# mayursharma/PageRank-using-Apache-Spark

Measured on AMD Instinct MI355X. Metric: PageRank GTEPS/iter + % HBM roofline, R-MAT scale-26 at 1/2/4/8 MI355X, higher is better.
Workload: dtype f64

## Files before the change

### pagerank-using-apache-spark_amd/csrc/pr_spmv.h

```cpp
#pragma once

#include <climits>

#include "pr_device.h"
#include "pr_internal.h"

namespace pr {

__device__ __forceinline__ double dc_from_slots(const double *cin, const SlotPos &sp) {
  double dc = 0.0;
  for (int p = 0; p < sp.n; ++p) dc = __dadd_rn(dc, cin[sp.pos[p]]);
  return dc;
}

__device__ __forceinline__ double affine(double S, double tdc, double teleport, double damping) {
  return __dadd_rn(teleport, __dmul_rn(damping, __dadd_rn(S, tdc)));
}

typedef int pr_v4i __attribute__((ext_vector_type(4)));
typedef int pr_v2i __attribute__((ext_vector_type(2)));
typedef pr_v4i pr_v4i_alias __attribute__((may_alias));
typedef uint32_t pr_u32_alias __attribute__((may_alias));
typedef double pr_f64_alias __attribute__((may_alias));

template <int PT, bool NT>
__device__ __forceinline__ void load_cols(const int32_t *__restrict__ p, int32_t (&ci)[PT]) {
  static_assert(PT % 4 == 0, "PT must be a multiple of 4");
  const pr_v4i *q = reinterpret_cast<const pr_v4i *>(p);
#pragma unroll
  for (int k = 0; k < PT / 4; ++k) {
    pr_v4i x;
    if constexpr (NT) x = __builtin_nontemporal_load(q + k);
    else x = q[k];
    ci[4 * k + 0] = x.x;
    ci[4 * k + 1] = x.y;
    ci[4 * k + 2] = x.z;
    ci[4 * k + 3] = x.w;
  }
}

template <int PT, bool NT, bool TELE>
__global__ __launch_bounds__(kThreads) void k_spmv_units(
    const Unit *__restrict__ units, const int64_t *__restrict__ rowptr,
    const int32_t *__restrict__ colp, const double *__restrict__ cin, double *__restrict__ cout,
    double *__restrict__ r, const uint32_t *__restrict__ rowinfo, double *__restrict__ piece_part,
    double2 *__restrict__ unit_part, SlotPos sp, int64_t S_pad, double n_vertices, double teleport,
    double damping, const double *__restrict__ tele) {
  __shared__ double rowsum[kUnitRows];
  __shared__ int32_t lrp[kUnitRows + 1];
  __shared__ double red[kThreads / kWave];
  __shared__ double2 red2[kThreads / kWave];
  __shared__ int32_t wrow_first[kThreads / kWave], wrow_last[kThreads / kWave];
  __shared__ double wval_last[kThreads / kWave];

  const int t = threadIdx.x, lane = lane_id(), w = wave_id();
  const Unit u = units[blockIdx.x];
  const int n = unit_n(u);
  const int i0 = t * PT;
  const bool stream = u.meta >= 0;
  const int nr = stream ? u.meta : 0;
  const int32_t r0 = u.r0;

  int32_t ci[PT];
  if (i0 < n) {
    load_cols<PT, NT>(colp + (int64_t)u.p8 * 8 + i0, ci);
  } else {
#pragma unroll
    for (int j = 0; j < PT; ++j) ci[j] = 0;
  }
  int64_t rp_t = 0;
  double rold0 = 0.0, tele0 = teleport;
  uint32_t info0 = 0;
  if (stream) {
    if (t <= nr) rp_t = rowptr[r0 + t];
    if (t < nr) {
      rold0 = r[(int64_t)r0 + t];
      info0 = rowinfo[(int64_t)r0 + t];
      if constexpr (TELE) tele0 = tele[(int64_t)r0 + t];
    }
  }

  double v[PT];
#pragma unroll
  for (int j = 0; j < PT; ++j) v[j] = (i0 + j < n) ? cin[ci[j]] : 0.0;

  if (!stream) {
    double acc = 0.0;
#pragma unroll
    for (int j = 0; j < PT; ++j) acc = __dadd_rn(acc, v[j]);
    acc = block_sum<kThreads>(acc, red);
    if (t == 0) {
      piece_part[-u.meta - 1] = acc;
      unit_part[blockIdx.x] = make_double2(0.0, 0.0);
    }
    return;
  }

  const int64_t e0 = rowptr[r0];
  if (t <= nr) lrp[t] = (int32_t)(rp_t - e0);
  for (int k = t + kThreads; k <= nr; k += kThreads) lrp[k] = (int32_t)(rowptr[r0 + k] - e0);
  const double tdc = dc_from_slots(cin, sp) / n_vertices;
  __syncthreads();

  int carry_row = -1, first_row = -1;
  double carry_val = 0.0, first_sum = 0.0;
  if (i0 < n) {
    int lo = 0, hi = nr + 1;
    while (lo < hi) {
      const int mid = (lo + hi) >> 1;
      if (lrp[mid] <= i0) lo = mid + 1;
      else hi = mid;
    }
    int cur = lo - 1;
    const int kstart = cur;
    const bool started_before = lrp[cur] < i0;
    int next_end = lrp[cur + 1];
    double acc = 0.0;
    bool open = false;
#pragma unroll
    for (int j = 0; j < PT; ++j) {
      if (i0 + j < n) {
        acc = __dadd_rn(acc, v[j]);
        open = true;
        if (i0 + j + 1 == next_end) {
          if (cur == kstart && started_before) {
            first_row = cur;
            first_sum = acc;
          } else {
            rowsum[cur] = acc;
          }
          acc = 0.0;
          open = false;
          ++cur;
          while (cur < nr && lrp[cur + 1] == lrp[cur]) ++cur;
          next_end = (cur < nr) ? lrp[cur + 1] : INT_MAX;
        }
      }
    }
    if (open) {
      carry_row = cur;
      carry_val = acc;
    }
  }

  int srow = carry_row;
  double sval = carry_val;
#pragma unroll
  for (int off = 1; off < kWave; off <<= 1) {
    const int prow = __shfl_up(srow, off, kWave);
    const double pval = __shfl_up(sval, off, kWave);
    if (lane >= off && srow >= 0 && prow == srow) sval = __dadd_rn(pval, sval);
  }
  const int lane0_row = __shfl(carry_row, 0, kWave);
  if (lane == kWave - 1) {
    wrow_last[w] = srow;
    wval_last[w] = sval;
    wrow_first[w] = lane0_row;
  }
  __syncthreads();
  int prow_in = -1;
  double pval_in = 0.0;
  for (int ww = 0; ww < w; ++ww) {
    const int rl = wrow_last[ww];
    const bool full = (rl >= 0) && (wrow_first[ww] == rl);
    if (full && prow_in == rl) {
      pval_in = __dadd_rn(pval_in, wval_last[ww]);
    } else {
      prow_in = rl;
      pval_in = (rl >= 0) ? wval_last[ww] : 0.0;
    }
  }
  if (srow >= 0 && srow == prow_in && lane0_row == srow) sval = __dadd_rn(pval_in, sval);
  int erow = __shfl_up(srow, 1, kWave);
  double eval = __shfl_up(sval, 1, kWave);
  if (lane == 0) {
    erow = prow_in;
    eval = pval_in;
  }
  if (first_row >= 0) rowsum[first_row] = (erow == first_row) ? __dadd_rn(eval, first_sum) : first_sum;
  __syncthreads();

  double dcp = 0.0, l1p = 0.0;
  for (int k = t; k < nr; k += kThreads) {
    const int64_t vtx = (int64_t)r0 + k;
    const double rold = (k == t) ? rold0 : r[vtx];
    const uint32_t info = (k == t) ? info0 : rowinfo[vtx];
    if (info & kRowHole) continue;
    const double S = (lrp[k + 1] > lrp[k]) ? rowsum[k] : rold;
    double tv = teleport;
    if constexpr (TELE) tv = (k == t) ? tele0 : tele[vtx];
    const double rn = affine(S, tdc, tv, damping);
    r[vtx] = rn;
    const uint32_t d = info & kRowDegMask;
    if (d > 0) cout[vtx] = __ddiv_rn(rn, (double)d);
    else if (info & kRowSink) dcp = __dadd_rn(dcp, rn);
    l1p = __dadd_rn(l1p, fabs(rn - rold));
  }
  const double2 part = block_sum2<kThreads>(make_double2(dcp, l1p), red2);
  if (t == 0) unit_part[blockIdx.x] = part;
}


template <int CTRL>
__device__ __forceinline__ double dpp_f64(double x) {
  const pr_v2i v = __builtin_bit_cast(pr_v2i, x);
  pr_v2i r;
  r.x = __builtin_amdgcn_update_dpp(0, v.x, CTRL, 0xF, 0xF, true);
  r.y = __builtin_amdgcn_update_dpp(0, v.y, CTRL, 0xF, 0xF, true);
  return __builtin_bit_cast(double, r);
}

template <int CTRL>
__device__ __forceinline__ int dpp_i32(int x) {
  return __builtin_amdgcn_update_dpp(0, x, CTRL, 0xF, 0xF, true);
}

__device__ __forceinline__ int wave_incl_scan_i32(int x) {
  const int row = lane_id() >> 4;
  x += dpp_i32<0x111>(x);
  x += dpp_i32<0x112>(x);
  x += dpp_i32<0x114>(x);
  x += dpp_i32<0x118>(x);
  int p = dpp_i32<0x142>(x);
  if (row == 1 || row == 3) x += p;
  p = dpp_i32<0x143>(x);
  if (row >= 2) x += p;
  return x;
}

__device__ __forceinline__ int wave_incl_max_i32(int x) {
  const int row = lane_id() >> 4;
  x = max(x, dpp_i32<0x111>(x));
  x = max(x, dpp_i32<0x112>(x));
  x = max(x, dpp_i32<0x114>(x));
  x = max(x, dpp_i32<0x118>(x));
  int p = dpp_i32<0x142>(x);
  if (row == 1 || row == 3) x = max(x, p);
  p = dpp_i32<0x143>(x);
  if (row >= 2) x = max(x, p);
  return x;
}

struct WaveCodes {
  uint32_t c[kWavePT];
};

__device__ __forceinline__ void wave_unit_codes(const Unit &u, const uint32_t *__restrict__ colh, WaveCodes &w) {
  const __amdgpu_buffer_rsrc_t rs =
      __builtin_amdgcn_make_buffer_rsrc((void *)(colh + (int64_t)u.p8 * 8), 0, u.n * 4, 0x00020000);
  const int base = lane_id() * kWavePT * 4;
#pragma unroll
  for (int q = 0; q < kWavePT / 4; ++q) {
    const pr_v4i x = __builtin_bit_cast(pr_v4i, __builtin_amdgcn_raw_buffer_load_b128(rs, base + 16 * q, 0, 2));
    w.c[4 * q + 0] = (uint32_t)x.x;
    w.c[4 * q + 1] = (uint32_t)x.y;
    w.c[4 * q + 2] = (uint32_t)x.z;
    w.c[4 * q + 3] = (uint32_t)x.w;
  }
}

struct WaveCodesC20 {
  uint32_t w[kWavePT / 2];
  uint32_t s;
};
__device__ __forceinline__ void wave_unit_codes(const Unit &u, const uint16_t *__restrict__ code16,
                                                const uint32_t *__restrict__ cside, WaveCodesC20 &w) {
  const __amdgpu_buffer_rsrc_t rm =
      __builtin_amdgcn_make_buffer_rsrc((void *)(code16 + (int64_t)u.p8 * 8), 0, u.n * 2, 0x00020000);
  const __amdgpu_buffer_rsrc_t rsd =
      __builtin_amdgcn_make_buffer_rsrc((void *)(cside + (int64_t)u.p8), 0, u.n / 2, 0x00020000);
  const pr_v4i x = __builtin_bit_cast(pr_v4i, __builtin_amdgcn_raw_buffer_load_b128(rm, lane_id() * 16, 0, 2));
  w.w[0] = (uint32_t)x.x;
  w.w[1] = (uint32_t)x.y;
  w.w[2] = (uint32_t)x.z;
  w.w[3] = (uint32_t)x.w;
  w.s = __builtin_amdgcn_raw_buffer_load_b32(rsd, lane_id() * 4, 0, 2);
}

struct WaveCodesC24 {
  uint32_t w[kWavePT / 2];
  uint64_t s;
};
__device__ __forceinline__ void wave_unit_codes(const Unit &u, const uint16_t *__restrict__ code16,
                                                const uint64_t *__restrict__ cside, WaveCodesC24 &w) {
  const __amdgpu_buffer_rsrc_t rm =
      __builtin_amdgcn_make_buffer_rsrc((void *)(code16 + (int64_t)u.p8 * 8), 0, u.n * 2, 0x00020000);
  const __amdgpu_buffer_rsrc_t rsd =
      __builtin_amdgcn_make_buffer_rsrc((void *)(cside + (int64_t)u.p8), 0, u.n, 0x00020000);
  const pr_v4i x = __builtin_bit_cast(pr_v4i, __builtin_amdgcn_raw_buffer_load_b128(rm, lane_id() * 16, 0, 2));
  w.w[0] = (uint32_t)x.x;
  w.w[1] = (uint32_t)x.y;
  w.w[2] = (uint32_t)x.z;
  w.w[3] = (uint32_t)x.w;
  w.s = __builtin_bit_cast(uint64_t, __builtin_amdgcn_raw_buffer_load_b64(rsd, lane_id() * 8, 0, 2));
}

__device__ __forceinline__ uint32_t end_marks(const WaveCodes &w) {
  uint32_t endm = 0;
#pragma unroll
  for (int j = 0; j < kWavePT; ++j) endm |= (w.c[j] & 1u) << j;
  return endm;
}
__device__ __forceinline__ uint32_t end_marks(const WaveCodesC20 &w) { return w.s & 0xFFu; }
__device__ __forceinline__ uint32_t end_marks(const WaveCodesC24 &w) { return (uint32_t)w.s & 0xFFu; }

struct LaneMeta {
  uint32_t endm;
  int excl;
  bool c[6];
};
__device__ __forceinline__ LaneMeta derive_meta(uint32_t endm) {
  LaneMeta m;
  m.endm = endm;
  const int t = lane_id(), r = t & 15, row = t >> 4;
  const int last1 = wave_incl_max_i32(endm ? t + 1 : 0);
  const int d = t + 1 - last1;
  const int dr = min(d, r);
#pragma unroll
  for (int s = 0; s < 4; ++s) m.c[s] = dr >= (1 << s);
  m.c[4] = (row & 1) && d > r;
  m.c[5] = row >= 2 && d > t - 32;
  const int cnt = __builtin_popcount(endm);
  m.excl = wave_incl_scan_i32(cnt) - cnt;
  return m;
}

struct ClassSrc {
  __amdgpu_buffer_rsrc_t crs;
  uint32_t zb, hb;
  const uint32_t *tbl;
};

template <bool PIECE>
__device__ __forceinline__ uint32_t cold_offset(uint32_t b8, const ClassSrc &cs) {
  if constexpr (PIECE) return piece_cold_offset(b8, cs.hb, cs.tbl);
  else return b8 - cs.hb;
}

#ifndef PR_GATHER_AUX
#define PR_GATHER_AUX 0
#endif
#ifndef PR_HOT_DIAG
#define PR_HOT_DIAG 0
#endif

template <bool PIECE>
__device__ __forceinline__ void wave_unit_gather(const WaveCodes &w, const double *hot, const ClassSrc &cs,
                                                 double (&v)[kWavePT]) {
#pragma unroll
  for (int j = 0; j < kWavePT; ++j) {
    const uint32_t c = w.c[j] & ~1u;
    const uint32_t la = (int32_t)c < 0 ? 0u : c;
    const double a = *reinterpret_cast<const double *>(reinterpret_cast<const char *>(hot) + la);
    const uint32_t go = c ^ kEntGlobal;
    const double b = __builtin_bit_cast(double, __builtin_amdgcn_raw_buffer_load_b64(cs.crs, go, 0, PR_GATHER_AUX));
    v[j] = __dadd_rn(a, b);
  }
}
template <bool PIECE>
__device__ __forceinline__ void wave_unit_gather(const WaveCodesC20 &w, const double *hot, const ClassSrc &cs,
                                                 double (&v)[kWavePT]) {
#pragma unroll
  for (int j = 0; j < kWavePT; ++j) {
    const uint32_t lo = (j & 1) ? (w.w[j >> 1] >> 16) : (w.w[j >> 1] & 0xFFFFu);
    const uint32_t idx = lo | (((w.s >> (8 + 3 * j)) & 7u) << 16);
    const uint32_t b8 = idx << 3;
    const uint32_t la = min(b8, cs.zb);
    const double a = *reinterpret_cast<const double *>(reinterpret_cast<const char *>(hot) + la);
#if PR_HOT_DIAG == 1
    const double b = __builtin_bit_cast(double, __builtin_amdgcn_raw_buffer_load_b64(cs.crs, cold_offset<PIECE>(b8, cs) | kEntGlobal, 0, PR_GATHER_AUX));
#elif PR_HOT_DIAG == 2 || PR_HOT_DIAG == 6
    const double b = 0.0;
#elif PR_HOT_DIAG == 3
    const uint32_t off = cold_offset<PIECE>(b8, cs);
    const double b = __dadd_rn(__builtin_bit_cast(double, __builtin_amdgcn_raw_buffer_load_b64(cs.crs, off, 0, PR_GATHER_AUX)),
                               __builtin_bit_cast(double, __builtin_amdgcn_raw_buffer_load_b64(cs.crs, off | kEntGlobal, 0, PR_GATHER_AUX)));
#else
    const double b = __builtin_bit_cast(double, __builtin_amdgcn_raw_buffer_load_b64(cs.crs, cold_offset<PIECE>(b8, cs), 0, PR_GATHER_AUX));
#endif
    v[j] = __dadd_rn(a, b);
  }
}

template <bool PIECE>
__device__ __forceinline__ void entry_addr(const WaveCodes &w, int j, const ClassSrc &, uint32_t &la, uint32_t &go) {
  const uint32_t c = w.c[j] & ~1u;
  la = (int32_t)c < 0 ? 0u : c;
  go = c ^ kEntGlobal;
}
template <bool PIECE>
__device__ __forceinline__ void entry_addr(const WaveCodesC20 &w, int j, const ClassSrc &cs, uint32_t &la, uint32_t &go) {
  const uint32_t lo = (j & 1) ? (w.w[j >> 1] >> 16) : (w.w[j >> 1] & 0xFFFFu);
  const uint32_t b8 = (lo | (((w.s >> (8 + 3 * j)) & 7u) << 16)) << 3;
  la = min(b8, cs.zb);
  go = cold_offset<PIECE>(b8, cs);
}
template <bool PIECE>
__device__ __forceinline__ void entry_addr(const WaveCodesC24 &w, int j, const ClassSrc &cs, uint32_t &la, uint32_t &go) {
  const uint32_t lo = (j & 1) ? (w.w[j >> 1] >> 16) : (w.w[j >> 1] & 0xFFFFu);
  const uint32_t b8 = (lo | ((uint32_t)(w.s >> (8 + 4 * j)) & 15u) << 16) << 3;
  la = min(b8, cs.zb);
  go = cold_offset<PIECE>(b8, cs);
}

static_assert(kStageSlots >= 2 * kWave, "the compact gather window holds 128 values (256 offsets)");
template <bool PIECE, class WC>
__device__ __forceinline__ void wave_unit_gather_compact(const WC &w, const double *hot, const ClassSrc &cs,
                                                         double (&v)[kWavePT], double *win) {
  uint32_t off[kWavePT], la[kWavePT];
  uint32_t coldm = 0u;
#pragma unroll
  for (int j = 0; j < kWavePT; ++j) {
    entry_addr<PIECE>(w, j, cs, la[j], off[j]);
    coldm |= ((int32_t)off[j] >= 0 ? 1u : 0u) << j;
  }
#pragma unroll
  for (int j = 0; j < kWavePT; ++j) v[j] = *reinterpret_cast<const double *>(reinterpret_cast<const char *>(hot) + la[j]);
  const int cnt = __builtin_popcount(coldm);
  const int incl = wave_incl_scan_i32(cnt);
  const int excl = incl - cnt, total = __builtin_amdgcn_readlane(incl, kWave - 1);
  const int lane = lane_id();
  pr_u32_alias *win32 = reinterpret_cast<pr_u32_alias *>(win);
  pr_f64_alias *winf = reinterpret_cast<pr_f64_alias *>(win);
  for (int base = 0; base < total; base += 4 * kWave) {
    int rk = excl - base;
#pragma unroll
    for (int j = 0; j < kWavePT; ++j) {
      const bool c = (coldm >> j) & 1u;
      if (c && (uint32_t)rk < (uint32_t)(4 * kWave)) win32[rk] = off[j];
      rk += c ? 1 : 0;
    }
    const int n = min(4 * kWave, total - base);
    const uint32_t a0 = lane < n ? win32[lane] : kEntGlobal;
    const uint32_t a1 = lane + kWave < n ? win32[lane + kWave] : kEntGlobal;
    const uint32_t a2 = lane + 2 * kWave < n ? win32[lane + 2 * kWave] : kEntGlobal;
    const uint32_t a3 = lane + 3 * kWave < n ? win32[lane + 3 * kWave] : kEntGlobal;
    const double g0 = __builtin_bit_cast(double, __builtin_amdgcn_raw_buffer_load_b64(cs.crs, a0, 0, PR_GATHER_AUX));
    double g1 = 0.0, g2 = 0.0, g3 = 0.0;
    if (n > kWave) g1 = __builtin_bit_cast(double, __builtin_amdgcn_raw_buffer_load_b64(cs.crs, a1, 0, PR_GATHER_AUX));
    if (n > 2 * kWave) g2 = __builtin_bit_cast(double, __builtin_amdgcn_raw_buffer_load_b64(cs.crs, a2, 0, PR_GATHER_AUX));
    if (n > 3 * kWave) g3 = __builtin_bit_cast(double, __builtin_amdgcn_raw_buffer_load_b64(cs.crs, a3, 0, PR_GATHER_AUX));
    winf[lane] = g0;
    if (n > kWave) winf[lane + kWave] = g1;
    rk = excl - base;
#pragma unroll
    for (int j = 0; j < kWavePT; ++j) {
      const bool c = (coldm >> j) & 1u;
      if (c && (uint32_t)rk < (uint32_t)(2 * kWave)) v[j] = winf[rk];
      rk += c ? 1 : 0;
    }
    if (n > 2 * kWave) {
      winf[lane] = g2;
      if (n > 3 * kWave) winf[lane + kWave] = g3;
      rk = excl - base - 2 * kWave;
#pragma unroll
      for (int j = 0; j < kWavePT; ++j) {
        const bool c = (coldm >> j) & 1u;
        if (c && (uint32_t)rk < (uint32_t)(2 * kWave)) v[j] = winf[rk];
        rk += c ? 1 : 0;
      }
    }
  }
}

template <bool PIECE>
__device__ __forceinline__ void wave_unit_gather(const WaveCodesC24 &w, const double *hot, const ClassSrc &cs,
                                                 double (&v)[kWavePT]) {
#pragma unroll
  for (int j = 0; j < kWavePT; ++j) {
    const uint32_t lo = (j & 1) ? (w.w[j >> 1] >> 16) : (w.w[j >> 1] & 0xFFFFu);
    const uint32_t idx = lo | ((uint32_t)(w.s >> (8 + 4 * j)) & 15u) << 16;
    const uint32_t b8 = idx << 3;
    const uint32_t la = min(b8, cs.zb);
    const double a = *reinterpret_cast<const double *>(reinterpret_cast<const char *>(hot) + la);
    const double b = __builtin_bit_cast(double, __builtin_amdgcn_raw_buffer_load_b64(cs.crs, cold_offset<PIECE>(b8, cs), 0, PR_GATHER_AUX));
    v[j] = __dadd_rn(a, b);
  }
}

__device__ __forceinline__ void wave_segmented_sums(const LaneMeta &m, const double (&v)[kWavePT],
                                                    double (&sv)[kWavePT], double *carry) {
  double acc = 0.0;
#pragma unroll
  for (int j = 0; j < kWavePT; ++j) {
    acc = __dadd_rn(acc, v[j]);
    sv[j] = acc;
    if (m.endm & (1u << j)) acc = 0.0;
  }
  double a = acc, p;
  p = dpp_f64<0x111>(a);
  if (m.c[0]) a = __dadd_rn(p, a);
  p = dpp_f64<0x112>(a);
  if (m.c[1]) a = __dadd_rn(p, a);
  p = dpp_f64<0x114>(a);
  if (m.c[2]) a = __dadd_rn(p, a);
  p = dpp_f64<0x118>(a);
  if (m.c[3]) a = __dadd_rn(p, a);
  p = dpp_f64<0x142>(a);
  if (m.c[4]) a = __dadd_rn(p, a);
  p = dpp_f64<0x143>(a);
  if (m.c[5]) a = __dadd_rn(p, a);
  *carry = dpp_f64<0x138>(a);
}

__device__ __forceinline__ void stage_segment_sums(const LaneMeta &m, const double (&sv)[kWavePT], double carry,
                                                   int base, double *stage) {
  int e = m.excl - base;
#pragma unroll
  for (int j = 0; j < kWavePT; ++j) {
    const bool end = (m.endm >> j) & 1u;
    if (end && e >= 0 && e < kStageSlots) stage[e] = sv[j];
    e += end ? 1 : 0;
  }
  const int e0 = m.excl - base;
  if (m.endm != 0u && e0 >= 0 && e0 < kStageSlots) stage[e0] = __dadd_rn(carry, stage[e0]);
}


struct UnitSums {
  LaneMeta m;
  double sv[kWavePT];
  double carry;
};

template <class WC>
__device__ __forceinline__ bool wave_unit_sums(const Unit &u, const WC &w, const double (&v)[kWavePT],
                                               double *__restrict__ piece_part, UnitSums &r) {
  if (u.meta < 0) {
    double acc = 0.0;
#pragma unroll
    for (int j = 0; j < kWavePT; ++j) acc = __dadd_rn(acc, v[j]);
    acc = wave_sum(acc);
    if (lane_id() == 0) piece_part[-u.meta - 1] = acc;
    return false;
  }
  r.m = derive_meta(end_marks(w));
  wave_segmented_sums(r.m, v, r.sv, &r.carry);
  return true;
}

__device__ __forceinline__ void wave_unit_store(const Unit &u, const UnitSums &r, double *pcls, double *stage) {
  const int nseg = u.meta;
  static_assert(kStageSlots <= 2 * kWave, "one b128 pass");
  const __amdgpu_buffer_rsrc_t urs =
      __builtin_amdgcn_make_buffer_rsrc((void *)(pcls + u.r0), 0, (uint32_t)nseg * 8u, 0x00020000);
  for (int base = 0; base < nseg; base += kStageSlots) {
    stage_segment_sums(r.m, r.sv, r.carry, base, stage);
    const int n = min(kStageSlots, nseg - base);
    const int i2 = 2 * lane_id();
#if PR_HOT_DIAG == 4 || PR_HOT_DIAG == 6
    if (u.r0 != 0x7FFFFFFF) continue;
#endif
    if (i2 < n)
      __builtin_amdgcn_raw_buffer_store_b128(*reinterpret_cast<const pr_v4i_alias *>(stage + i2), urs,
                                             (uint32_t)(base + i2) * 8u, 0, 2);
  }
}

struct CodeSrc {
  const void *codes;
  const uint32_t *side;
};
template <int CODE>
struct CodeOf {
  using T = WaveCodes;
};
template <>
struct CodeOf<kCodeC20> {
  using T = WaveCodesC20;
};
template <>
struct CodeOf<kCodeC24> {
  using T = WaveCodesC24;
};
template <>
struct CodeOf<kCodeC20P> {
  using T = WaveCodesC20;
};
template <>
struct CodeOf<kCodeC24P> {
  using T = WaveCodesC24;
};
template <int CODE>
__device__ __forceinline__ void unit_codes(const Unit &u, const CodeSrc &cd, typename CodeOf<CODE>::T &w) {
  if constexpr (CODE == kCodeC20 || CODE == kCodeC20P)
    wave_unit_codes(u, static_cast<const uint16_t *>(cd.codes), cd.side, w);
  else if constexpr (CODE == kCodeC24 || CODE == kCodeC24P)
    wave_unit_codes(u, static_cast<const uint16_t *>(cd.codes), reinterpret_cast<const uint64_t *>(cd.side), w);
  else wave_unit_codes(u, static_cast<const uint32_t *>(cd.codes), w);
}

template <int CODE, bool DENSE>
__device__ __forceinline__ void unit_gather(const typename CodeOf<CODE>::T &w, const double *hot, const ClassSrc &cs,
                                            double (&v)[kWavePT], double *win) {
  if constexpr (DENSE && (!PR_HOT_DIAG || PR_HOT_DIAG == 7)) {
    wave_unit_gather_compact<code_is_piece(CODE)>(w, hot, cs, v, win);
  } else {
    (void)win;
    wave_unit_gather<code_is_piece(CODE)>(w, hot, cs, v);
  }
}

template <int CODE, bool DENSE>
__device__ __forceinline__ void hot_class_units(int x, int team, int nteams, const Unit *__restrict__ units,
                                                const int64_t *__restrict__ ucum, const HotGeom &hg,
                                                const CodeSrc &cd, const double *hot, const ClassSrc &cs,
                                                double *__restrict__ partial, const int64_t *__restrict__ poff,
                                                double *__restrict__ piece_part, double *stage) {
  const int64_t p0 = poff[x];
  const int64_t beg = ucum[x], end = ucum[x + 1];
  constexpr int kWaves = kHotThreads / kWave;
  team = (team + 5 * (x / kXcds)) % nteams;
  const int64_t stride = (int64_t)nteams * kWaves;
  uint32_t *ctr = reinterpret_cast<uint32_t *>(const_cast<double *>(hot) + hg.ctr_slot());
  const int lane = lane_id();
  auto counter = [&]() -> uint32_t {
    uint32_t t = 0;
    if (lane == 0) t = atomicAdd(ctr, 1u);
    return (uint32_t)__builtin_amdgcn_readlane((int)t, 0);
  };
  auto take = [&]() -> int64_t {
    const uint32_t t = counter();
    return beg + (int64_t)team * kWaves + (int64_t)(t % kWaves) + (int64_t)(t / kWaves) * stride;
  };
  int64_t k = take();
  if (k >= end) return;
  const __attribute__((address_space(4))) pr_v4i *cu = (const __attribute__((address_space(4))) pr_v4i *)units;
  auto unit_at = [&](int64_t i) -> Unit {
    const pr_v4i q = cu[i];
    return Unit{(uint32_t)q.x, q.y, q.z, q.w};
  };
  const int64_t none_k = ucum[kMaxClasses];
  Unit u[3];
  typename CodeOf<CODE>::T wc[3];
  double v[3][kWavePT];
  int64_t k1 = take();
  u[0] = unit_at(k);
  unit_codes<CODE>(u[0], cd, wc[0]);
  u[1] = unit_at(k1 < end ? k1 : none_k);
  unit_codes<CODE>(u[1], cd, wc[1]);
  unit_gather<CODE, DENSE>(wc[0], hot, cs, v[0], stage);
  while (true) {
#pragma unroll
    for (int sl = 0; sl < 3; ++sl) {
      const int s1 = (sl + 1) % 3, s2 = (sl + 2) % 3;
      const int64_t k2 = take();
      u[s2] = unit_at(k2 < end ? k2 : none_k);
      unit_codes<CODE>(u[s2], cd, wc[s2]);
#if PR_HOT_DIAG == 7
      {
        uint32_t d = (uint32_t)lane;
#pragma unroll
        for (int q = 0; q < 64; ++q) asm volatile("v_add_u32 %0, %0, %1" : "+v"(d) : "v"((uint32_t)q));
        if (d == 0xFFFFFFFFu) piece_part[0] = 0.0;
      }
#endif
      UnitSums us;
      const bool stream = wave_unit_sums(u[sl], wc[sl], v[sl], piece_part, us);
      if (stream) wave_unit_store(u[sl], us, partial + p0, stage);
      unit_gather<CODE, DENSE>(wc[s1], hot, cs, v[s1], stage);
      k = k1;
      k1 = k2;
      if (k >= end) return;
    }
  }
}

template <bool PIECE, bool CONTIG = false>
__device__ __forceinline__ void stage_hot_set(const HotGeom &hg, int x, const int32_t *__restrict__ hpos,
                                              const int32_t *__restrict__ ptab, const double *__restrict__ cin,
                                              double *hot, uint32_t *tblw) {
  const int nh = hg.P * hg.Kp;
  const int32_t *hp = hpos + (int64_t)x * nh;
  const double *reg = cin + (int64_t)x * hg.Q_pad;
  const bool load = PR_HOT_DIAG != 5 || x < kXcds;
  constexpr int kSB = 6;
  for (int b0 = 0; load && b0 < nh; b0 += kSB * kHotThreads) {
    int32_t pos[kSB];
    double val[kSB];
    if constexpr (CONTIG) {
#pragma unroll
      for (int j = 0; j < kSB; ++j) {
        const int i = b0 + (int)threadIdx.x + j * kHotThreads;
        val[j] = i < hg.q_load ? reg[i] : 0.0;
      }
    } else {
#pragma unroll
      for (int j = 0; j < kSB; ++j) {
        const int i = b0 + (int)threadIdx.x + j * kHotThreads;
        pos[j] = i < nh ? hp[i] : -1;
      }
#pragma unroll
      for (int j = 0; j < kSB; ++j) val[j] = pos[j] >= 0 ? cin[pos[j]] : 0.0;
    }
#pragma unroll
    for (int j = 0; j < kSB; ++j) {
      const int i = b0 + (int)threadIdx.x + j * kHotThreads;
      if (i < nh) hot[1 + i] = val[j];
    }
  }
  if constexpr (PIECE)
    for (int i = (int)threadIdx.x; i < kPieceTblWords; i += kHotThreads)
      tblw[i] = (uint32_t)ptab[(int64_t)x * kPieceTblWords + i];
  if (threadIdx.x == 0) {
    hot[0] = 0.0;
    hot[hg.slots()] = 0.0;
    *reinterpret_cast<uint32_t *>(hot + hg.ctr_slot()) = 0u;
  }
}

template <int CODE, bool DENSE>
__global__ __launch_bounds__(kHotThreads) void k_spmv_hot(const Unit *__restrict__ units,
                                                          const int64_t *__restrict__ ucum, HotGeom hg,
                                                          CodeSrc cd, const double *__restrict__ cin,
                                                          uint32_t cin_bytes, double *__restrict__ partial,
                                                          const int64_t *__restrict__ poff,
                                                          double *__restrict__ piece_part,
                                                          const int32_t *__restrict__ hpos,
                                                          const int32_t *__restrict__ ptab, int ph0, int ph1) {
  __shared__ double hot[kHotLdsBytes / sizeof(double)];
  constexpr bool kPiece = code_is_piece(CODE);
  ClassSrc cs;
  cs.zb = (uint32_t)hg.slots() * 8u;
  cs.hb = kPiece ? cs.zb : (uint32_t)(hg.q_load + 1) * 8u;
  uint32_t *tblw = reinterpret_cast<uint32_t *>(hot + hg.tbl_off());
  cs.tbl = tblw;
  if constexpr (CODE == kCodeU32 || kPiece)
    cs.crs = __builtin_amdgcn_make_buffer_rsrc((void *)cin, 0, cin_bytes, 0x00020000);
  const int wv = __builtin_amdgcn_readfirstlane(wave_id());
  double *stage = hot + hg.stage_off() + wv * kStageSlots;
  const int team = (int)(blockIdx.x / kXcds), nteams = (int)(gridDim.x / kXcds);
  for (int ph = ph0; ph < ph1; ++ph) {
    const int x = (int)(blockIdx.x % kXcds) + kXcds * ph;
    if constexpr (CODE == kCodeC20 || CODE == kCodeC24) {
      const int64_t first = (int64_t)x * hg.Q_pad + hg.q_load;
      cs.crs = __builtin_amdgcn_make_buffer_rsrc((void *)(cin + first), 0,
                                                 (uint32_t)((hg.Q_pad - hg.q_load) * 8), 0x00020000);
    }
    if (ph > ph0) __syncthreads();
    stage_hot_set<kPiece, CODE == kCodeC20 || CODE == kCodeC24>(hg, x, hpos, ptab, cin, hot, tblw);
    __syncthreads();
    hot_class_units<CODE, DENSE>(x, team, nteams, units, ucum, hg, cd, hot, cs, partial, poff, piece_part, stage);
  }
}

__global__ __launch_bounds__(kThreads) void k_seg_reduce(int64_t n_seg, const int64_t *__restrict__ seg_slot,
                                                         const int32_t *__restrict__ seg_p0,
                                                         const double *__restrict__ piece_part,
                                                         double *__restrict__ partial) {
  const int lane = lane_id();
  const int64_t nw = (int64_t)gridDim.x * (kThreads / kWave);
  for (int64_t q = (int64_t)blockIdx.x * (kThreads / kWave) + wave_id(); q < n_seg; q += nw) {
    const int32_t p0 = seg_p0[q], np = seg_p0[q + 1] - p0;
    double acc = 0.0;
    for (int k = lane; k < np; k += kWave) acc = __dadd_rn(acc, piece_part[p0 + k]);
    acc = wave_sum(acc);
    if (lane == 0) partial[seg_slot[q]] = acc;
  }
}

template <int G>
__device__ __forceinline__ int epi_class_add(const uint32_t (&mw)[G], uint32_t bit, int run, const double *win,
                                             int zslot, double (&S)[G]) {
  double v[G];
#pragma unroll
  for (int g = 0; g < G; ++g) {
    const bool has = (mw[g] & bit) != 0u;
    const unsigned long long bal = __ballot(has);
    const int idx = (int)__builtin_amdgcn_mbcnt_hi((uint32_t)(bal >> 32),
                                                   __builtin_amdgcn_mbcnt_lo((uint32_t)bal, (uint32_t)run));
    v[g] = win[has ? idx : zslot];
    run += __popcll(bal);
  }
#pragma unroll
  for (int g = 0; g < G; ++g) S[g] = __dadd_rn(S[g], v[g]);
  return run;
}

template <int C, int W>
__device__ __forceinline__ int walk_batch_end(int x0, int incl, int pre, int sincl, int spre) {
  static_assert(W >= 64 * kEpiGroup + 2 + 2 * 8 * kEpiGroup, "one class and its positions fit the window");
  const int lane = lane_id();
  const int base = __builtin_amdgcn_readlane(pre, x0), sbase = __builtin_amdgcn_readlane(spre, x0);
  const int need = (incl - base) + 2 * ((sincl - sbase + 7) >> 3);
  const unsigned long long over = __ballot(lane >= x0 && lane < C && need > W);
  return over ? (int)__builtin_ctzll(over) : C;
}
__device__ __forceinline__ uint64_t class_range_mask(int x0, int x1) {
  const uint64_t hi = x1 >= 64 ? ~0ull : ((1ull << x1) - 1ull);
  return hi & ~((1ull << x0) - 1ull);
}


struct EpiArgs {
  int64_t nblk;
  const double *partial;
  const void *rmask;
  const int32_t *cbase;
  const uint32_t *rowinfo;
  double *r, *cout;
  double teleport, damping;
  const int64_t *eoff;
  const uint16_t *epos;
  const uint8_t *pmask;
  const int32_t *sbase;
  const double *tele;
};

#ifndef PR_EPI_DMA_AUX
#define PR_EPI_DMA_AUX 0
#endif
#ifndef PR_EPI_LATE_ROW
#define PR_EPI_LATE_ROW 0
#endif
#ifndef PR_EPI_TELE_EARLY
#define PR_EPI_TELE_EARLY 0
#endif

template <int C, bool WALK, bool TELE>
__device__ __forceinline__ void epi_group(const EpiArgs &a, const PackDst &pd, int64_t gi, double tdc, double *win,
                                          double2 *__restrict__ ep_part) {
  double dcp = 0.0, l1p = 0.0;
  constexpr int G = kEpiGroup, W = kEpiWin;
  constexpr int MW = mask_words<C>();
  static_assert(MW == 1 || MW == 2 || MW == 4, "mask words");
  static_assert(W >= 64 * G + 2, "one class run of a group must fit the window");
  static_assert(!WALK || C <= kWave, "the per-row walk needs at most 64 classes");
  const int lane = lane_id();
  const int64_t b0 = gi * G;
  const int nb = (int)min((int64_t)G, a.nblk - b0);
  uint32_t mw[MW][G], info[G];
  double rold[G], S[G];
  double tv[G];
  double cnv[G];
  uint32_t pmv[G];
#pragma unroll
  for (int g = 0; g < G; ++g) pmv[g] = (pd.P > 1 && g < nb) ? a.pmask[(b0 + g) * kWave + lane] : 0u;
#pragma unroll
  for (int g = 0; g < G; ++g) {
    const int64_t L = (b0 + g) * kWave + lane;
    const bool ok = g < nb;
    if constexpr (MW == 4) {
      const uint4 q = ok ? static_cast<const uint4 *>(a.rmask)[L] : make_uint4(0u, 0u, 0u, 0u);
      mw[0][g] = q.x, mw[1][g] = q.y, mw[2][g] = q.z, mw[3][g] = q.w;
    } else if constexpr (MW == 2) {
      const uint2 q = ok ? static_cast<const uint2 *>(a.rmask)[L] : make_uint2(0u, 0u);
      mw[0][g] = q.x, mw[1][g] = q.y;
    } else {
      mw[0][g] = ok ? static_cast<const uint32_t *>(a.rmask)[L] : 0u;
    }
#if !PR_EPI_LATE_ROW
    info[g] = ok ? a.rowinfo[L] : kRowHole;
    rold[g] = ok ? a.r[L] : 0.0;
#endif
#if PR_EPI_TELE_EARLY
    if constexpr (TELE) tv[g] = ok ? a.tele[L] : 0.0;
#endif
    S[g] = 0.0;
  }
  const int cs = lane < C ? a.cbase[b0 * C + lane] : 0;
  const int ce = lane < C ? a.cbase[(b0 + nb) * C + lane] : 0;
  if constexpr (C <= kWave) {
    const int sa = cs & ~1;
    const int n2 = (lane < C && ce > cs) ? (((ce + 1) & ~1) - sa) : 0;
    const int incl = wave_incl_scan_i32(n2);
    const int pre = incl - n2;
    const int roff = incl - n2 + (cs - sa);
    bool walked = false;
    if constexpr (WALK) {
      const int64_t eo = a.eoff[gi];
      if (eo >= 0) {
        const int nsl = lane < C ? ce - cs : 0;
        const int sincl = wave_incl_scan_i32(nsl);
        for (int y = 0; y < C; ++y) {
          const int n = __builtin_amdgcn_readlane(n2, y);
          if (n == 0) continue;
          const double *src = a.partial + __builtin_amdgcn_readlane(sa, y);
          double *dst = win + __builtin_amdgcn_readlane(pre, y);
          for (int o = 0; o < n; o += 2 * kWave)
            if (o + 2 * lane < n) __builtin_amdgcn_global_load_lds(src + o + 2 * lane, dst + o, 16, 0, PR_EPI_DMA_AUX);
        }
        const int Tb = __builtin_amdgcn_readlane(incl, C - 1);
        const int nl = (__builtin_amdgcn_readlane(sincl, C - 1) + 7) >> 3;
        const double *esrc = reinterpret_cast<const double *>(a.epos + eo);
        for (int o = 0; o < nl; o += kWave)
          if (o + lane < nl) __builtin_amdgcn_global_load_lds(esrc + 2 * (o + lane), win + Tb + 2 * o, 16, 0, PR_EPI_DMA_AUX);
        __builtin_amdgcn_s_waitcnt(0);
        const uint16_t *ep = reinterpret_cast<const uint16_t *>(win + Tb);
        int acc = 0;
#pragma unroll
        for (int g = 0; g < G; ++g) {
          const uint64_t m = (uint64_t)(MW > 1 ? mw[MW > 1 ? 1 : 0][g] : 0u) << 32 | mw[0][g];
          const int cnt = __popcll(m);
          const int inc = wave_incl_scan_i32(cnt);
          const uint16_t *e = ep + acc + inc - cnt;
          acc += __builtin_amdgcn_readlane(inc, kWave - 1);
          for (int k = 0; __ballot(k < cnt) != 0ull; ++k)
            if (k < cnt) S[g] = __dadd_rn(S[g], win[e[k]]);
        }
        __builtin_amdgcn_s_waitcnt(0);
        walked = true;
      }
    }
    for (int x0 = 0; x0 < C && !walked;) {
      const int base = __builtin_amdgcn_readlane(pre, x0);
      const unsigned long long over = __ballot(lane >= x0 && lane < C && incl - base > W);
      const int x1 = over ? (int)__builtin_ctzll(over) : C;
      for (int y = x0; y < x1; ++y) {
        const int n = __builtin_amdgcn_readlane(n2, y);
        if (n == 0) continue;
        const double *src = a.partial + __builtin_amdgcn_readlane(sa, y);
        double *dst = win + (__builtin_amdgcn_readlane(pre, y) - base);
        for (int o = 0; o < n; o += 2 * kWave)
          if (o + 2 * lane < n) __builtin_amdgcn_global_load_lds(src + o + 2 * lane, dst + o, 16, 0, PR_EPI_DMA_AUX);
      }
      __builtin_amdgcn_s_waitcnt(0);
      for (int y = x0; y < x1; ++y) {
        if (__builtin_amdgcn_readlane(n2, y) == 0) continue;
        const uint32_t bit = 1u << (y & 31);
        const int run = __builtin_amdgcn_readlane(roff, y) - base;
        if (MW == 1 || y < 32) epi_class_add<G>(mw[0], bit, run, win, W, S);
        else epi_class_add<G>(mw[MW > 1 ? 1 : 0], bit, run, win, W, S);
      }
      __builtin_amdgcn_s_waitcnt(0);
      x0 = x1;
    }
  } else {
    const int cs1 = lane + kWave < C ? a.cbase[b0 * C + kWave + lane] : 0;
    const int ce1 = lane + kWave < C ? a.cbase[(b0 + nb) * C + kWave + lane] : 0;
    auto run_start = [&](int y) {
      return y < kWave ? __builtin_amdgcn_readlane(cs, y) : __builtin_amdgcn_readlane(cs1, y - kWave);
    };
    auto run_end = [&](int y) {
      return y < kWave ? __builtin_amdgcn_readlane(ce, y) : __builtin_amdgcn_readlane(ce1, y - kWave);
    };
    for (int x = 0; x < C;) {
      int fill = 0, xe = x;
      for (; xe < C; ++xe) {
        const int s = run_start(xe), e = run_end(xe);
        if (e == s) continue;
        const int sa = s & ~1, n2 = ((e + 1) & ~1) - sa;
        if (xe > x && fill + n2 > W) break;
        const double *src = a.partial + sa;
        for (int o = 0; o < n2; o += 2 * kWave)
          if (o + 2 * lane < n2) __builtin_amdgcn_global_load_lds(src + o + 2 * lane, win + fill + o, 16, 0, PR_EPI_DMA_AUX);
        fill += n2;
      }
      __builtin_amdgcn_s_waitcnt(0);
      fill = 0;
      for (int y = x; y < xe; ++y) {
        const int s = run_start(y), e = run_end(y);
        if (e == s) continue;
        const int sa = s & ~1;
        const uint32_t bit = 1u << (y & 31);
        const int run = fill + (s - sa);
        if (y < 32) epi_class_add<G>(mw[0], bit, run, win, W, S);
        else if (y < 64) epi_class_add<G>(mw[MW > 1 ? 1 : 0], bit, run, win, W, S);
        else if (y < 96) epi_class_add<G>(mw[MW > 2 ? 2 : 0], bit, run, win, W, S);
        else epi_class_add<G>(mw[MW > 3 ? 3 : 0], bit, run, win, W, S);
        fill += ((e + 1) & ~1) - sa;
      }
      __builtin_amdgcn_s_waitcnt(0);
      x = xe;
    }
  }
#if PR_EPI_LATE_ROW
#pragma unroll
  for (int g = 0; g < G; ++g) {
    const int64_t L = (b0 + g) * kWave + lane;
    const bool ok = g < nb;
    info[g] = ok ? a.rowinfo[L] : kRowHole;
    rold[g] = ok ? a.r[L] : 0.0;
  }
#endif
#pragma unroll
  for (int g = 0; g < G; ++g) {
    const int64_t L = (b0 + g) * kWave + lane;
    if constexpr (!TELE) tv[g] = a.teleport;
#if !PR_EPI_TELE_EARLY
    else tv[g] = g < nb ? a.tele[L] : 0.0;
#endif
    double Sv = S[g];
    uint32_t any = 0u;
#pragma unroll
    for (int w = 0; w < MW; ++w) any |= mw[w][g];
    if (any == 0u) Sv = rold[g];
    const double rn = affine(Sv, tdc, tv[g], a.damping);
    double cn = 0.0;
    if (!(info[g] & kRowHole)) {
      a.r[L] = rn;
      const uint32_t d = info[g] & kRowDegMask;
      if (d > 0) {
        cn = __ddiv_rn(rn, (double)d);
        a.cout[L] = cn;
      } else if (info[g] & kRowSink) {
        dcp = __dadd_rn(dcp, rn);
      }
      l1p = __dadd_rn(l1p, fabs(rn - rold[g]));
    }
    cnv[g] = cn;
  }
  static_assert(G * kWave <= W, "a group's run for one peer fits the window");
  if (pd.P > 1) {
    const int64_t sb0 = b0 * pd.P;
    for (int q = 0; q < pd.P; ++q) {
      int run = 0;
#pragma unroll
      for (int g = 0; g < G; ++g) {
        const bool has = (pmv[g] >> q) & 1u;
        const unsigned long long bal = __ballot(has);
        const int k = (int)__builtin_amdgcn_mbcnt_hi((uint32_t)(bal >> 32), __builtin_amdgcn_mbcnt_lo((uint32_t)bal, (uint32_t)run));
        if (has) win[k] = cnv[g];
        run += __popcll(bal);
      }
      if (run == 0) continue;
      const __amdgpu_buffer_rsrc_t rs = __builtin_amdgcn_make_buffer_rsrc(
          (void *)(pd.sbuf + pd.soff[q] + a.sbase[sb0 + q]), 0, (uint32_t)run * 8u, 0x00020000);
      for (int o = 0; o < run; o += 2 * kWave) {
        const int i = o + 2 * lane;
        if (i < run)
          __builtin_amdgcn_raw_buffer_store_b128(*reinterpret_cast<const pr_v4i_alias *>(win + i), rs, (uint32_t)i * 8u, 0, 0);
      }
    }
  }
  dcp = wave_sum(dcp);
  l1p = wave_sum(l1p);
  if (lane == 0) ep_part[gi] = make_double2(dcp, l1p);
}

#ifndef PR_EPI_WAVES
#define PR_EPI_WAVES 0
#endif
#if PR_EPI_WAVES > 0
#define PR_EPI_BOUNDS(NT) __attribute__((amdgpu_flat_work_group_size(NT, NT), amdgpu_waves_per_eu(PR_EPI_WAVES)))
#else
#define PR_EPI_BOUNDS(NT) __launch_bounds__(NT, 4)
#endif
template <int C, bool WALK, int NT, bool TELE>
__global__ PR_EPI_BOUNDS(NT) void k_epilogue_grp(
    int64_t nblk, int64_t g_lo, int64_t g_hi, const double *__restrict__ partial, const void *__restrict__ rmask_v,
    const int32_t *__restrict__ cbase, const uint32_t *__restrict__ rowinfo, double *__restrict__ r,
    double *__restrict__ cout, const double *__restrict__ cin, SlotPos sp, double n_vertices, double teleport,
    double damping, double2 *__restrict__ ep_part , const int64_t *__restrict__ eoff,
    const uint16_t *__restrict__ epos, const uint8_t *__restrict__ pmask, const int32_t *__restrict__ sbase,
    const int32_t *__restrict__ order, PackDst pd, const double *__restrict__ tele) {
  constexpr int W = kEpiWin;
  constexpr int NW = NT / kWave;
  extern __shared__ double epi_lds[];
  const EpiArgs a{nblk, partial, rmask_v, cbase, rowinfo, r, cout, teleport, damping, eoff, epos, pmask, sbase, tele};
  const int lane = lane_id();
  const int wv = __builtin_amdgcn_readfirstlane(wave_id());
  double *win = epi_lds + wv * (W + 2);
  if (lane == 0) win[W] = 0.0;
  const double tdc = dc_from_slots(cin, sp) / n_vertices;
  const int64_t nw = (int64_t)gridDim.x * NW;
  for (int64_t k = g_lo + (int64_t)blockIdx.x * NW + wv; k < g_hi; k += nw)
    epi_group<C, WALK, TELE>(a, pd, order ? (int64_t)order[k] : k, tdc, win, ep_part);
}

template <int C, bool COUNT>
__global__ __launch_bounds__(kEpiThreads) void k_epi_walk_plan(int64_t nblk, const void *__restrict__ rmask_v,
                                                               const int32_t *__restrict__ cbase,
                                                               int64_t *__restrict__ eoff,
                                                               uint16_t *__restrict__ epos) {
  static_assert(C <= kWave, "per-row walk: at most 64 classes");
  constexpr int G = kEpiGroup, W = kEpiWin;
  constexpr int MW = mask_words<C>();
  const int lane = lane_id();
  const int64_t ngrp = (nblk + G - 1) / G;
  const int64_t nw = (int64_t)gridDim.x * (kEpiThreads / kWave);
  for (int64_t gi = (int64_t)blockIdx.x * (kEpiThreads / kWave) + wave_id(); gi < ngrp; gi += nw) {
    int64_t ebase = 0;
    if constexpr (!COUNT) {
      ebase = eoff[gi];
      if (ebase < 0) continue;
    }
    const int64_t b0 = gi * G;
    const int nb = (int)min((int64_t)G, nblk - b0);
    uint64_t m[G];
#pragma unroll
    for (int g = 0; g < G; ++g) {
      const int64_t L = (b0 + g) * kWave + lane;
      if (g >= nb) m[g] = 0;
      else if constexpr (MW == 2) m[g] = static_cast<const uint64_t *>(rmask_v)[L];
      else m[g] = static_cast<const uint32_t *>(rmask_v)[L];
    }
    const int cs = lane < C ? cbase[b0 * C + lane] : 0;
    const int ce = lane < C ? cbase[(b0 + nb) * C + lane] : 0;
    const int sa = cs & ~1;
    const int n2 = (lane < C && ce > cs) ? (((ce + 1) & ~1) - sa) : 0;
    const int incl = wave_incl_scan_i32(n2);
    const int pre = incl - n2;
    const int roff = pre + (cs - sa);
    const int nsl = lane < C ? ce - cs : 0;
    const int sincl = wave_incl_scan_i32(nsl);
    const int spre = sincl - nsl;
    const int x1 = walk_batch_end<C, W>(0, incl, pre, sincl, spre);
    const int nl = (__builtin_amdgcn_readlane(sincl, x1 - 1) + 7) >> 3;
    if constexpr (COUNT) {
      if (lane == 0) eoff[gi] = x1 == C ? 8 * (int64_t)nl : -1;
    } else {
      int pref[G], acc = 0;
#pragma unroll
      for (int g = 0; g < G; ++g) {
        const int cnt = __popcll(m[g]);
        const int inc = wave_incl_scan_i32(cnt);
        pref[g] = acc + inc - cnt;
        acc += __builtin_amdgcn_readlane(inc, kWave - 1);
      }
      for (int x = 0; x < C; ++x) {
        int run = __builtin_amdgcn_readlane(roff, x);
#pragma unroll
        for (int g = 0; g < G; ++g) {
          const bool has = (m[g] >> x) & 1ull;
          const unsigned long long bal = __ballot(has);
          if (has) {
            const int k = __popcll(m[g] & ((1ull << x) - 1ull));
            epos[ebase + pref[g] + k] = (uint16_t)__builtin_amdgcn_mbcnt_hi(
                (uint32_t)(bal >> 32), __builtin_amdgcn_mbcnt_lo((uint32_t)bal, (uint32_t)run));
          }
          run += __popcll(bal);
        }
      }
    }
  }
}

using EpiGrpFn = void (*)(int64_t, int64_t, int64_t, const double *, const void *, const int32_t *, const uint32_t *, double *,
                          double *, const double *, SlotPos, double, double, double, double2 *, const int64_t *,
                          const uint16_t *, const uint8_t *, const int32_t *, const int32_t *, PackDst, const double *);
template <int C, bool TELE>
inline EpiGrpFn epi_grp_kernel_c(bool walk, bool narrow) {
  if constexpr (C <= kWave) {
    if (narrow)
      return walk ? k_epilogue_grp<C, true, kEpiThreadsNarrow, TELE> : k_epilogue_grp<C, false, kEpiThreadsNarrow, TELE>;
    if (walk) return k_epilogue_grp<C, true, kEpiThreads, TELE>;
  }
  return k_epilogue_grp<C, false, kEpiThreads, TELE>;
}
template <bool TELE>
inline EpiGrpFn epi_grp_kernel_t(int C, bool walk, bool narrow) {
  switch (C) {
    case 8: return epi_grp_kernel_c<8, TELE>(walk, narrow);
    case 16: return epi_grp_kernel_c<16, TELE>(walk, narrow);
    case 32: return epi_grp_kernel_c<32, TELE>(walk, narrow);
    case 64: return epi_grp_kernel_c<64, TELE>(walk, narrow);
    default: return epi_grp_kernel_c<128, TELE>(false, false);
  }
}
inline EpiGrpFn epi_grp_kernel(int C, bool walk, bool narrow, bool tele = false) {
  return tele ? epi_grp_kernel_t<true>(C, walk, narrow) : epi_grp_kernel_t<false>(C, walk, narrow);
}

}
```

Baseline: 382.4.

## Fuse wave scans, ballot segment ends, and move unit counter to LDS atomics

Packs the cold-entry count and the segment-end count into one wave prefix scan during the compact gather, and reuses the end-exclusive offset in the segmented sums so the second scan is skipped. The incl-max DPP scan is replaced by a ballot plus count-leading-zeros. Per-entry rank keys are precomputed once, so the gather and stage loops avoid repeated running-rank arithmetic, and the accumulator reset becomes a branchless mask. The work counter is cast to an LDS address and updated with a workgroup-scope relaxed atomic, with 32-bit indices. Packing both counts into 16-bit halves of one scan limits each to 65535 per wave, and the LDS cast assumes the counter slot really lives in shared memory.

```diff
diff --git a/pagerank-using-apache-spark_amd/csrc/pr_spmv.h b/pagerank-using-apache-spark_amd/csrc/pr_spmv.h
--- a/pagerank-using-apache-spark_amd/csrc/pr_spmv.h
+++ b/pagerank-using-apache-spark_amd/csrc/pr_spmv.h
@@ -228,19 +228,6 @@
   return x;
 }
 
-__device__ __forceinline__ int wave_incl_max_i32(int x) {
-  const int row = lane_id() >> 4;
-  x = max(x, dpp_i32<0x111>(x));
-  x = max(x, dpp_i32<0x112>(x));
-  x = max(x, dpp_i32<0x114>(x));
-  x = max(x, dpp_i32<0x118>(x));
-  int p = dpp_i32<0x142>(x);
-  if (row == 1 || row == 3) x = max(x, p);
-  p = dpp_i32<0x143>(x);
-  if (row >= 2) x = max(x, p);
-  return x;
-}
-
 struct WaveCodes {
   uint32_t c[kWavePT];
 };
@@ -309,19 +296,24 @@
   int excl;
   bool c[6];
 };
+template <bool SCAN = true>
 __device__ __forceinline__ LaneMeta derive_meta(uint32_t endm) {
   LaneMeta m;
   m.endm = endm;
   const int t = lane_id(), r = t & 15, row = t >> 4;
-  const int last1 = wave_incl_max_i32(endm ? t + 1 : 0);
+  const unsigned long long bal = __ballot(endm != 0u);
+  const int last1 = 64 - __clzll((long long)(bal & ((2ull << t) - 1ull)));
   const int d = t + 1 - last1;
   const int dr = min(d, r);
 #pragma unroll
   for (int s = 0; s < 4; ++s) m.c[s] = dr >= (1 << s);
   m.c[4] = (row & 1) && d > r;
   m.c[5] = row >= 2 && d > t - 32;
-  const int cnt = __builtin_popcount(endm);
-  m.excl = wave_incl_scan_i32(cnt) - cnt;
+  m.excl = 0;
+  if constexpr (SCAN) {
+    const int cnt = __builtin_popcount(endm);
+    m.excl = wave_incl_scan_i32(cnt) - cnt;
+  }
   return m;
 }
 
@@ -406,30 +398,33 @@
 static_assert(kStageSlots >= 2 * kWave, "the compact gather window holds 128 values (256 offsets)");
 template <bool PIECE, class WC>
 __device__ __forceinline__ void wave_unit_gather_compact(const WC &w, const double *hot, const ClassSrc &cs,
-                                                         double (&v)[kWavePT], double *win) {
-  uint32_t off[kWavePT], la[kWavePT];
-  uint32_t coldm = 0u;
+                                                         double (&v)[kWavePT], double *win, int *end_excl) {
+  uint32_t off[kWavePT], key[kWavePT];
+  int cnt = 0;
 #pragma unroll
   for (int j = 0; j < kWavePT; ++j) {
-    entry_addr<PIECE>(w, j, cs, la[j], off[j]);
-    coldm |= ((int32_t)off[j] >= 0 ? 1u : 0u) << j;
-  }
-#pragma unroll
-  for (int j = 0; j < kWavePT; ++j) v[j] = *reinterpret_cast<const double *>(reinterpret_cast<const char *>(hot) + la[j]);
-  const int cnt = __builtin_popcount(coldm);
-  const int incl = wave_incl_scan_i32(cnt);
-  const int excl = incl - cnt, total = __builtin_amdgcn_readlane(incl, kWave - 1);
+    uint32_t la;
+    entry_addr<PIECE>(w, j, cs, la, off[j]);
+    v[j] = *reinterpret_cast<const double *>(reinterpret_cast<const char *>(hot) + la);
+    key[j] = (off[j] & kEntGlobal) | (uint32_t)cnt;
+    cnt += 1 + ((int32_t)off[j] >> 31);
+  }
+  const int ends = __builtin_popcount(end_marks(w));
+  const int both = cnt | (ends << 16);
+  const int incl2 = wave_incl_scan_i32(both);
+  *end_excl = (incl2 - both) >> 16;
+  const int incl = incl2 & 0xFFFF;
+  const int excl = incl - cnt, total = __builtin_amdgcn_readlane(incl2, kWave - 1) & 0xFFFF;
+  if (total == 0) return;
+#pragma unroll
+  for (int j = 0; j < kWavePT; ++j) key[j] += (uint32_t)excl;
   const int lane = lane_id();
   pr_u32_alias *win32 = reinterpret_cast<pr_u32_alias *>(win);
   pr_f64_alias *winf = reinterpret_cast<pr_f64_alias *>(win);
-  for (int base = 0; base < total; base += 4 * kWave) {
-    int rk = excl - base;
-#pragma unroll
-    for (int j = 0; j < kWavePT; ++j) {
-      const bool c = (coldm >> j) & 1u;
-      if (c && (uint32_t)rk < (uint32_t)(4 * kWave)) win32[rk] = off[j];
-      rk += c ? 1 : 0;
-    }
+  for (int base = 0;;) {
+#pragma unroll
+    for (int j = 0; j < kWavePT; ++j)
+      if (key[j] < (uint32_t)(4 * kWave)) win32[key[j]] = off[j];
     const int n = min(4 * kWave, total - base);
     const uint32_t a0 = lane < n ? win32[lane] : kEntGlobal;
     const uint32_t a1 = lane + kWave < n ? win32[lane + kWave] : kEntGlobal;
@@ -442,24 +437,20 @@
     if (n > 3 * kWave) g3 = __builtin_bit_cast(double, __builtin_amdgcn_raw_buffer_load_b64(cs.crs, a3, 0, PR_GATHER_AUX));
     winf[lane] = g0;
     if (n > kWave) winf[lane + kWave] = g1;
-    rk = excl - base;
-#pragma unroll
-    for (int j = 0; j < kWavePT; ++j) {
-      const bool c = (coldm >> j) & 1u;
-      if (c && (uint32_t)rk < (uint32_t)(2 * kWave)) v[j] = winf[rk];
-      rk += c ? 1 : 0;
-    }
+#pragma unroll
+    for (int j = 0; j < kWavePT; ++j)
+      if (key[j] < (uint32_t)(2 * kWave)) v[j] = winf[key[j]];
     if (n > 2 * kWave) {
       winf[lane] = g2;
       if (n > 3 * kWave) winf[lane + kWave] = g3;
-      rk = excl - base - 2 * kWave;
-#pragma unroll
-      for (int j = 0; j < kWavePT; ++j) {
-        const bool c = (coldm >> j) & 1u;
-        if (c && (uint32_t)rk < (uint32_t)(2 * kWave)) v[j] = winf[rk];
-        rk += c ? 1 : 0;
-      }
-    }
+#pragma unroll
+      for (int j = 0; j < kWavePT; ++j)
+        if (key[j] - (uint32_t)(2 * kWave) < (uint32_t)(2 * kWave)) v[j] = winf[key[j] - 2 * kWave];
+    }
+    base += 4 * kWave;
+    if (base >= total) break;
+#pragma unroll
+    for (int j = 0; j < kWavePT; ++j) key[j] -= (uint32_t)(4 * kWave);
   }
 }
 
@@ -478,6 +469,10 @@
   }
 }
 
+__device__ __forceinline__ uint32_t open_mask(uint32_t endm, int j) {
+  return (uint32_t)((int32_t)(~endm << (31 - j)) >> 31);
+}
+
 __device__ __forceinline__ void wave_segmented_sums(const LaneMeta &m, const double (&v)[kWavePT],
                                                     double (&sv)[kWavePT], double *carry) {
   double acc = 0.0;
@@ -485,7 +480,11 @@
   for (int j = 0; j < kWavePT; ++j) {
     acc = __dadd_rn(acc, v[j]);
     sv[j] = acc;
-    if (m.endm & (1u << j)) acc = 0.0;
+    pr_v2i a = __builtin_bit_cast(pr_v2i, acc);
+    const int open = (int)open_mask(m.endm, j);
+    a.x &= open;
+    a.y &= open;
+    acc = __builtin_bit_cast(double, a);
   }
   double a = acc, p;
   p = dpp_f64<0x111>(a);
@@ -503,29 +502,15 @@
   *carry = dpp_f64<0x138>(a);
 }
 
-__device__ __forceinline__ void stage_segment_sums(const LaneMeta &m, const double (&sv)[kWavePT], double carry,
-                                                   int base, double *stage) {
-  int e = m.excl - base;
-#pragma unroll
-  for (int j = 0; j < kWavePT; ++j) {
-    const bool end = (m.endm >> j) & 1u;
-    if (end && e >= 0 && e < kStageSlots) stage[e] = sv[j];
-    e += end ? 1 : 0;
-  }
-  const int e0 = m.excl - base;
-  if (m.endm != 0u && e0 >= 0 && e0 < kStageSlots) stage[e0] = __dadd_rn(carry, stage[e0]);
-}
-
-
 struct UnitSums {
   LaneMeta m;
   double sv[kWavePT];
   double carry;
 };
 
-template <class WC>
+template <bool SCAN, class WC>
 __device__ __forceinline__ bool wave_unit_sums(const Unit &u, const WC &w, const double (&v)[kWavePT],
-                                               double *__restrict__ piece_part, UnitSums &r) {
+                                               double *__restrict__ piece_part, UnitSums &r, int end_excl) {
   if (u.meta < 0) {
     double acc = 0.0;
 #pragma unroll
@@ -534,7 +519,8 @@
     if (lane_id() == 0) piece_part[-u.meta - 1] = acc;
     return false;
   }
-  r.m = derive_meta(end_marks(w));
+  r.m = derive_meta<SCAN>(end_marks(w));
+  if constexpr (!SCAN) r.m.excl = end_excl;
   wave_segmented_sums(r.m, v, r.sv, &r.carry);
   return true;
 }
@@ -544,8 +530,25 @@
   static_assert(kStageSlots <= 2 * kWave, "one b128 pass");
   const __amdgpu_buffer_rsrc_t urs =
       __builtin_amdgcn_make_buffer_rsrc((void *)(pcls + u.r0), 0, (uint32_t)nseg * 8u, 0x00020000);
-  for (int base = 0; base < nseg; base += kStageSlots) {
-    stage_segment_sums(r.m, r.sv, r.carry, base, stage);
+  uint32_t skey[kWavePT];
+  uint32_t e = (uint32_t)r.m.excl;
+#pragma unroll
+  for (int j = 0; j < kWavePT; ++j) {
+    const uint32_t open = open_mask(r.m.endm, j);
+    skey[j] = e | (open & kEntGlobal);
+    e += 1u + open;
+  }
+  uint32_t ckey = (uint32_t)r.m.excl | (r.m.endm != 0u ? 0u : kEntGlobal);
+  auto next_pass = [&]() {
+#pragma unroll
+    for (int j = 0; j < kWavePT; ++j) skey[j] -= (uint32_t)kStageSlots;
+    ckey -= (uint32_t)kStageSlots;
+  };
+  for (int base = 0; base < nseg; base += kStageSlots, next_pass()) {
+#pragma unroll
+    for (int j = 0; j < kWavePT; ++j)
+      if (skey[j] < (uint32_t)kStageSlots) stage[skey[j]] = r.sv[j];
+    if (ckey < (uint32_t)kStageSlots) stage[ckey] = __dadd_rn(r.carry, stage[ckey]);
     const int n = min(kStageSlots, nseg - base);
     const int i2 = 2 * lane_id();
 #if PR_HOT_DIAG == 4 || PR_HOT_DIAG == 6
@@ -592,10 +595,11 @@
 
 template <int CODE, bool DENSE>
 __device__ __forceinline__ void unit_gather(const typename CodeOf<CODE>::T &w, const double *hot, const ClassSrc &cs,
-                                            double (&v)[kWavePT], double *win) {
+                                            double (&v)[kWavePT], double *win, int *end_excl) {
   if constexpr (DENSE && (!PR_HOT_DIAG || PR_HOT_DIAG == 7)) {
-    wave_unit_gather_compact<code_is_piece(CODE)>(w, hot, cs, v, win);
+    wave_unit_gather_compact<code_is_piece(CODE)>(w, hot, cs, v, win, end_excl);
   } else {
+    (void)end_excl;
     (void)win;
     wave_unit_gather<code_is_piece(CODE)>(w, hot, cs, v);
   }
@@ -611,41 +615,44 @@
   const int64_t beg = ucum[x], end = ucum[x + 1];
   constexpr int kWaves = kHotThreads / kWave;
   team = (team + 5 * (x / kXcds)) % nteams;
-  const int64_t stride = (int64_t)nteams * kWaves;
-  uint32_t *ctr = reinterpret_cast<uint32_t *>(const_cast<double *>(hot) + hg.ctr_slot());
+  const uint32_t n_cls = (uint32_t)(end - beg), none_i = (uint32_t)(ucum[kMaxClasses] - beg);
+  const uint32_t first = (uint32_t)team * kWaves, stride = (uint32_t)nteams * kWaves;
   const int lane = lane_id();
-  auto counter = [&]() -> uint32_t {
-    uint32_t t = 0;
-    if (lane == 0) t = atomicAdd(ctr, 1u);
-    return (uint32_t)__builtin_amdgcn_readlane((int)t, 0);
+  typedef __attribute__((address_space(3))) uint32_t lds_u32;
+  uint32_t ctr_a = (uint32_t)(uintptr_t)(lds_u32 *)reinterpret_cast<uint32_t *>(const_cast<double *>(hot) + hg.ctr_slot());
+  asm volatile("" : "+v"(ctr_a));
+  auto take = [&]() -> uint32_t {
+    uint32_t tv = 0;
+    if (lane == 0)
+      tv = __hip_atomic_fetch_add((lds_u32 *)(uintptr_t)ctr_a, 1u, __ATOMIC_RELAXED, __HIP_MEMORY_SCOPE_WORKGROUP);
+    const uint32_t t = (uint32_t)__builtin_amdgcn_readlane((int)tv, 0);
+    return first + (t % kWaves) + (t / kWaves) * stride;
   };
-  auto take = [&]() -> int64_t {
-    const uint32_t t = counter();
-    return beg + (int64_t)team * kWaves + (int64_t)(t % kWaves) + (int64_t)(t / kWaves) * stride;
-  };
-  int64_t k = take();
-  if (k >= end) return;
-  const __attribute__((address_space(4))) pr_v4i *cu = (const __attribute__((address_space(4))) pr_v4i *)units;
-  auto unit_at = [&](int64_t i) -> Unit {
+  uint32_t k = take();
+  if (k >= n_cls) return;
+  const __attribute__((address_space(4))) pr_v4i *cu = (const __attribute__((address_space(4))) pr_v4i *)(units + beg);
+  auto unit_at = [&](uint32_t i) -> Unit {
     const pr_v4i q = cu[i];
     return Unit{(uint32_t)q.x, q.y, q.z, q.w};
   };
-  const int64_t none_k = ucum[kMaxClasses];
   Unit u[3];
   typename CodeOf<CODE>::T wc[3];
   double v[3][kWavePT];
-  int64_t k1 = take();
+  int end_excl[3] = {0, 0, 0};
+  constexpr bool kDenseGather = DENSE && (!PR_HOT_DIAG || PR_HOT_DIAG == 7);
+  constexpr bool kEndScan = !kDenseGather;
+  uint32_t k1 = take();
   u[0] = unit_at(k);
   unit_codes<CODE>(u[0], cd, wc[0]);
-  u[1] = unit_at(k1 < end ? k1 : none_k);
+  u[1] = unit_at(k1 < n_cls ? k1 : none_i);
   unit_codes<CODE>(u[1], cd, wc[1]);
-  unit_gather<CODE, DENSE>(wc[0], hot, cs, v[0], stage);
+  unit_gather<CODE, DENSE>(wc[0], hot, cs, v[0], stage, &end_excl[0]);
   while (true) {
 #pragma unroll
     for (int sl = 0; sl < 3; ++sl) {
       const int s1 = (sl + 1) % 3, s2 = (sl + 2) % 3;
-      const int64_t k2 = take();
-      u[s2] = unit_at(k2 < end ? k2 : none_k);
+      const uint32_t k2 = take();
+      u[s2] = unit_at(k2 < n_cls ? k2 : none_i);
       unit_codes<CODE>(u[s2], cd, wc[s2]);
 #if PR_HOT_DIAG == 7
       {
@@ -656,12 +663,12 @@
       }
 #endif
       UnitSums us;
-      const bool stream = wave_unit_sums(u[sl], wc[sl], v[sl], piece_part, us);
+      const bool stream = wave_unit_sums<kEndScan>(u[sl], wc[sl], v[sl], piece_part, us, end_excl[sl]);
       if (stream) wave_unit_store(u[sl], us, partial + p0, stage);
-      unit_gather<CODE, DENSE>(wc[s1], hot, cs, v[s1], stage);
+      unit_gather<CODE, DENSE>(wc[s1], hot, cs, v[s1], stage, &end_excl[s1]);
       k = k1;
       k1 = k2;
-      if (k >= end) return;
+      if (k >= n_cls) return;
     }
   }
 }
```

After: 367.5. -3.9%, worse.
